# Bill9125/T2MS

Hardware: AMD Instinct MI355X
Metric: generated series/sec (B=256, L=96, 1000-step DDPM) (higher is better)
Workload: dtype f32; 1 GPU; configs[1]: DiT denoiser, 1000-step ddpm with CFG (2 forwards/step), B=256/GPU, L=96, cfg_scale=9.0, LA-VAE decode; Philox noise on device; hipGraph=on; sampler lanes=2 (part-batch chains on own streams, include/t2s.h t2s_sampler_set_lanes); global_batch=256, diffusion_steps=1000, parallelism=batch-shard x1, sampler_lanes=2

## Files before the change

t2ms_amd/csrc/t2s_attn.hip:

```cpp
#include <stdlib.h>

#include "t2s_dit_internal.h"

namespace t2s {

struct SoftmaxState {
    float m_run;
    float l_lane;
};

__device__ __forceinline__ float pair_max(float v) {
    const auto r = __builtin_amdgcn_permlane32_swap(__float_as_uint(v), __float_as_uint(v), false, false);
    return fmaxf(__uint_as_float(r[0]), __uint_as_float(r[1]));
}
__device__ __forceinline__ float pair_sum(float v) {
    const auto r = __builtin_amdgcn_permlane32_swap(__float_as_uint(v), __float_as_uint(v), false, false);
    return __uint_as_float(r[0]) + __uint_as_float(r[1]);
}

__device__ __forceinline__ void softmax_block(f32x16& st, f32x16& ot, SoftmaxState& s) {
    float mloc = st[0];
#pragma unroll
    for (int r = 1; r < 16; ++r) mloc = fmaxf(mloc, st[r]);
    mloc = pair_max(mloc);
    const float m_new = fmaxf(s.m_run, mloc);
    const float alpha = __builtin_amdgcn_exp2f(s.m_run - m_new);
    s.m_run = m_new;
    float psum = 0.f;
#pragma unroll
    for (int r = 0; r < 16; ++r) {
        st[r] = __builtin_amdgcn_exp2f(st[r] - m_new);
        psum += st[r];
    }
    s.l_lane = s.l_lane * alpha + psum;
#pragma unroll
    for (int r = 0; r < 16; ++r) ot[r] *= alpha;
}

constexpr float QSCALE = 0.17677669529663687f * 1.4426950408889634f;

constexpr int ATT_SLOTS = 4;
constexpr int ATT_SLOT_F4 = 512;
constexpr int ATT_LDS_BYTES = ATT_SLOTS * ATT_SLOT_F4 * 16;
constexpr int NKB = NTOK / 32;

constexpr float SM_BIG = 1.152921504606847e18f;


struct TileState {
    f32x16 negm;
    float m_ref;
    float l_lane;
};

__device__ __forceinline__ float exp_sum(f32x16& st) {
#pragma unroll
    for (int r = 0; r < 16; ++r) st[r] = __builtin_amdgcn_exp2f(st[r]);
    return ((st[0] + st[1]) + (st[2] + st[3])) + ((st[4] + st[5]) + (st[6] + st[7])) +
           (((st[8] + st[9]) + (st[10] + st[11])) + ((st[12] + st[13]) + (st[14] + st[15])));
}

__device__ __forceinline__ float rereference(const f32x4 (&kf)[4], const f32x4 (&q)[4], f32x16& st,
                                             f32x16& ot, TileState& t) {
#pragma unroll
    for (int r = 0; r < 16; ++r) st[r] = 0.f;
#pragma unroll
    for (int g = 0; g < 4; ++g)
#pragma unroll
        for (int e = 0; e < 4; ++e) st = mfma32(kf[g][e], q[g][e], st);
    float mloc = st[0];
#pragma unroll
    for (int r = 1; r < 16; ++r) mloc = fmaxf(mloc, st[r]);
    mloc = pair_max(mloc);
    const float m_new = fmaxf(t.m_ref, mloc);
    const float alpha = __builtin_amdgcn_exp2f(t.m_ref - m_new);
    t.m_ref = m_new;
    t.l_lane *= alpha;
#pragma unroll
    for (int r = 0; r < 16; ++r) {
        ot[r] *= alpha;
        t.negm[r] = -m_new;
        st[r] -= m_new;
    }
    return exp_sum(st);
}

template <int NT, int NKBT>
__device__ __forceinline__ void attn_packed_body(f32x4* ring, const f32x4* qg, const f32x4* kg,
                                                 const f32x4* vg, f32x4* og, int bh, int t0, int lane,
                                                 int wave) {
    f32x4 qa[4], qb[4];
#pragma unroll
    for (int g = 0; g < 4; ++g) {
        qa[g] = qg[(t0 * 4 + g) * 64 + lane] * QSCALE;
        if (NT == 2) qb[g] = qg[((t0 + 1) * 4 + g) * 64 + lane] * QSCALE;
    }
    f32x16 oa, ob;
    TileState ta, tb;
#pragma unroll
    for (int r = 0; r < 16; ++r) {
        oa[r] = ob[r] = 0.f;
        ta.negm[r] = tb.negm[r] = INFINITY;
    }
    ta.m_ref = tb.m_ref = -INFINITY;
    ta.l_lane = tb.l_lane = 0.f;

    auto issue_clamped = [&](int jb) {
        const int src = jb < NKBT ? jb : NKBT - 1;
        f32x4* slot = ring + (jb & (ATT_SLOTS - 1)) * ATT_SLOT_F4;
        glds16_asm(kg + (src * 4 + wave) * 64 + lane, slot + wave * 64);
        glds16_asm(vg + (src * 4 + wave) * 64 + lane, slot + 256 + wave * 64);
    };
    asm volatile("s_waitcnt vmcnt(4)" ::: "memory");
    __builtin_amdgcn_s_barrier();
    issue_clamped(3);
    f32x4 kf[4];
#pragma unroll
    for (int g = 0; g < 4; ++g) kf[g] = ring[g * 64 + lane];

#pragma unroll 1
    for (int jb = 0; jb < NKBT; ++jb) {
        const f32x4* slot = ring + (jb & (ATT_SLOTS - 1)) * ATT_SLOT_F4 + lane;
        f32x4 vf[4];
#pragma unroll
        for (int g = 0; g < 4; ++g) vf[g] = slot[256 + g * 64];

        f32x16 sta = ta.negm, stb = tb.negm;
        float psa = 0.f, psb = 0.f;
        bool redo = jb == 0;
        if (!redo) {
            sta = mfma32_from(kf[0][0], qa[0][0], ta.negm);
            if (NT == 2) stb = mfma32_from(kf[0][0], qb[0][0], tb.negm);
#pragma unroll
            for (int g = 0; g < 4; ++g)
#pragma unroll
                for (int e = (g == 0 ? 1 : 0); e < 4; ++e) {
                    sta = mfma32(kf[g][e], qa[g][e], sta);
                    if (NT == 2) stb = mfma32(kf[g][e], qb[g][e], stb);
                }
            psa = exp_sum(sta);
            if (NT == 2) psb = exp_sum(stb);
            const bool stale = !(psa < SM_BIG) || !(psb < SM_BIG);
            redo = __builtin_amdgcn_ballot_w64(stale) != 0;
        }
        if (redo) {
            psa = rereference(kf, qa, sta, oa, ta);
            if (NT == 2) psb = rereference(kf, qb, stb, ob, tb);
        }
        ta.l_lane += psa;
        tb.l_lane += psb;
#pragma unroll
        for (int g = 0; g < 4; ++g)
#pragma unroll
            for (int e = 0; e < 4; ++e) oa = mfma32(vf[g][e], sta[4 * g + e], oa);
        asm volatile("s_waitcnt vmcnt(4)" ::: "memory");
        __builtin_amdgcn_s_barrier();
        issue_clamped(jb + 4);
        {
            const f32x4* nslot = ring + ((jb + 1) & (ATT_SLOTS - 1)) * ATT_SLOT_F4 + lane;
#pragma unroll
            for (int g = 0; g < 4; ++g) kf[g] = nslot[g * 64];
        }
        if (NT == 2) {
#pragma unroll
            for (int g = 0; g < 4; ++g)
#pragma unroll
                for (int e = 0; e < 4; ++e) ob = mfma32(vf[g][e], stb[4 * g + e], ob);
        }
    }
    asm volatile("s_waitcnt vmcnt(0)" ::: "memory");

    const int seq = bh / NH, head = bh % NH;
    {
        const float inv = 1.0f / pair_sum(ta.l_lane);
#pragma unroll
        for (int g = 0; g < 4; ++g) {
            const f32x4 w = {oa[4 * g] * inv, oa[4 * g + 1] * inv, oa[4 * g + 2] * inv, oa[4 * g + 3] * inv};
            og[(((size_t)seq * NKBT + t0) * 16 + head * 4 + g) * 64 + lane] = w;
        }
    }
    if (NT == 2) {
        const float inv = 1.0f / pair_sum(tb.l_lane);
#pragma unroll
        for (int g = 0; g < 4; ++g) {
            const f32x4 w = {ob[4 * g] * inv, ob[4 * g + 1] * inv, ob[4 * g + 2] * inv, ob[4 * g + 3] * inv};
            og[(((size_t)seq * NKBT + t0 + 1) * 16 + head * 4 + g) * 64 + lane] = w;
        }
    }
}

template <int PARTS, int TPW, int NKBT>
__device__ __forceinline__ void attn_packed_head(const float* __restrict__ q, const float* __restrict__ k,
                                                 const float* __restrict__ vT, float* __restrict__ o, int BH) {
    extern __shared__ __attribute__((aligned(16))) f32x4 ring[];
    const int grp = blockIdx.x / (8 * PARTS), rr = blockIdx.x % (8 * PARTS);
    const int bh = grp * 8 + (rr & 7);
    const int part = rr >> 3;
    if (bh >= BH) return;
    const int lane = threadIdx.x & 63;
    const int wave = __builtin_amdgcn_readfirstlane(threadIdx.x >> 6);
    const f32x4* qg = reinterpret_cast<const f32x4*>(q) + (size_t)bh * NKBT * 256;
    const f32x4* kg = reinterpret_cast<const f32x4*>(k) + (size_t)bh * NKBT * 256;
    const f32x4* vg = reinterpret_cast<const f32x4*>(vT) + (size_t)bh * NKBT * 256;
    f32x4* og = reinterpret_cast<f32x4*>(o);

    {
        f32x4* slot0 = ring;
        f32x4* slot1 = ring + ATT_SLOT_F4;
        glds16_asm(kg + (0 * 4 + wave) * 64 + lane, slot0 + wave * 64);
        glds16_asm(vg + (0 * 4 + wave) * 64 + lane, slot0 + 256 + wave * 64);
        glds16_asm(kg + (1 * 4 + wave) * 64 + lane, slot1 + wave * 64);
        glds16_asm(vg + (1 * 4 + wave) * 64 + lane, slot1 + 256 + wave * 64);
        f32x4* slot2 = ring + 2 * ATT_SLOT_F4;
        glds16_asm(kg + (2 * 4 + wave) * 64 + lane, slot2 + wave * 64);
        glds16_asm(vg + (2 * 4 + wave) * 64 + lane, slot2 + 256 + wave * 64);
    }
    if constexpr (TPW == 2) {
        const int t0 = part * 8 + wave * 2;
        if (t0 + 1 < NKBT) {
            attn_packed_body<2, NKBT>(ring, qg, kg, vg, og, bh, t0, lane, wave);
        } else if constexpr (PARTS * 8 > NKBT + 1) {
            attn_packed_body<1, NKBT>(ring, qg, kg, vg, og, bh, t0 < NKBT ? t0 : NKBT - 1, lane, wave);
        } else {
            attn_packed_body<1, NKBT>(ring, qg, kg, vg, og, bh, t0, lane, wave);
        }
    } else {
        const int t = part * 4 + wave;
        attn_packed_body<1, NKBT>(ring, qg, kg, vg, og, bh, t < NKBT ? t : NKBT - 1, lane, wave);
    }
}

template <int PARTS>
__global__ __launch_bounds__(256, 2) void attn_fwd_packed_kernel(const float* __restrict__ q,
                                                                 const float* __restrict__ k,
                                                                 const float* __restrict__ vT,
                                                                 float* __restrict__ o, int BH) {
    attn_packed_head<PARTS, PARTS == 2 ? 2 : 1, NKB>(q, k, vT, o, BH);
}

template <int NKBT>
__global__ __launch_bounds__(256, 2) void attn_fwd_packed_wide_kernel(const float* __restrict__ q,
                                                                      const float* __restrict__ k,
                                                                      const float* __restrict__ vT,
                                                                      float* __restrict__ o, int BH) {
    static_assert(NKBT > 24 && NKBT <= 32, "four workgroups of 8 tile slots");
    attn_packed_head<4, 2, NKBT>(q, k, vT, o, BH);
}

constexpr int PERSIST_THREADS = 512;

template <int NT>
__device__ __forceinline__ void attn_persistent_body(f32x4* ring, const f32x4* qall, const f32x4* kall,
                                                     const f32x4* vall, f32x4* og, int BH, int lane, int wave) {
    const int stride = gridDim.x;
    const int t0 = wave * 2;
    auto issue_block = [&](int bh, int jb, int gslot) {
        if constexpr (NT == 1) {
            if (jb >= NKB) { jb -= NKB; bh += stride; }
            if (bh >= BH) { bh -= stride; jb = NKB - 1; }
            const size_t off = (size_t)bh * NKB * 256 + jb * 4 * 64 + lane;
            f32x4* dst = ring + (gslot & (ATT_SLOTS - 1)) * ATT_SLOT_F4;
#pragma unroll
            for (int f = 0; f < 4; ++f) {
                glds16_asm(kall + off + f * 64, dst + f * 64);
                glds16_asm(vall + off + f * 64, dst + 256 + f * 64);
            }
        }
    };
#define ATT_PERSIST_WAIT() if constexpr (NT == 1) asm volatile("s_waitcnt vmcnt(16)" ::: "memory")
    int bh = blockIdx.x;
    int gb = 0;
    issue_block(bh, 0, 0);
    issue_block(bh, 1, 1);
    issue_block(bh, 2, 2);

    f32x4 qa[4], qb[4], qna[4], qnb[4];
    {
        const f32x4* qg = qall + (size_t)bh * NKB * 256;
#pragma unroll
        for (int g = 0; g < 4; ++g) {
            qa[g] = qg[(t0 * 4 + g) * 64 + lane] * QSCALE;
            if (NT == 2) qb[g] = qg[((t0 + 1) * 4 + g) * 64 + lane] * QSCALE;
            qna[g] = qa[g];
            qnb[g] = qb[g];
        }
    }
    ATT_PERSIST_WAIT();
    __builtin_amdgcn_s_barrier();
    issue_block(bh, 3, 3);
    f32x4 kf[4];
#pragma unroll
    for (int g = 0; g < 4; ++g) kf[g] = ring[g * 64 + lane];

#pragma unroll 1
    for (; bh < BH; bh += stride) {
        f32x16 oa, ob;
        TileState ta, tb;
#pragma unroll
        for (int r = 0; r < 16; ++r) {
            oa[r] = ob[r] = 0.f;
            ta.negm[r] = tb.negm[r] = INFINITY;
        }
        ta.m_ref = tb.m_ref = -INFINITY;
        ta.l_lane = tb.l_lane = 0.f;

#pragma unroll 1
        for (int jb = 0; jb < NKB; ++jb, ++gb) {
            const f32x4* slot = ring + (gb & (ATT_SLOTS - 1)) * ATT_SLOT_F4 + lane;
            f32x4 vf[4];
#pragma unroll
            for (int g = 0; g < 4; ++g) vf[g] = slot[256 + g * 64];
            f32x16 sta = ta.negm, stb = tb.negm;
            float psa = 0.f, psb = 0.f;
            bool redo = jb == 0;
            if (!redo) {
                sta = mfma32_from(kf[0][0], qa[0][0], ta.negm);
                if (NT == 2) stb = mfma32_from(kf[0][0], qb[0][0], tb.negm);
#pragma unroll
                for (int g = 0; g < 4; ++g)
#pragma unroll
                    for (int e = (g == 0 ? 1 : 0); e < 4; ++e) {
                        sta = mfma32(kf[g][e], qa[g][e], sta);
                        if (NT == 2) stb = mfma32(kf[g][e], qb[g][e], stb);
                    }
                psa = exp_sum(sta);
                if (NT == 2) psb = exp_sum(stb);
                const bool stale = !(psa < SM_BIG) || !(psb < SM_BIG);
                redo = __builtin_amdgcn_ballot_w64(stale) != 0;
            }
            if (redo) {
                psa = rereference(kf, qa, sta, oa, ta);
                if (NT == 2) psb = rereference(kf, qb, stb, ob, tb);
            }
            ta.l_lane += psa;
            tb.l_lane += psb;
#pragma unroll
            for (int g = 0; g < 4; ++g)
#pragma unroll
                for (int e = 0; e < 4; ++e) oa = mfma32(vf[g][e], sta[4 * g + e], oa);
            if (jb == NKB - 4 && bh + stride < BH) {
                const f32x4* qg = qall + (size_t)(bh + stride) * NKB * 256;
#pragma unroll
                for (int g = 0; g < 4; ++g) {
                    qna[g] = qg[(t0 * 4 + g) * 64 + lane];
                    if (NT == 2) qnb[g] = qg[((t0 + 1) * 4 + g) * 64 + lane];
                }
            }
            ATT_PERSIST_WAIT();
            __builtin_amdgcn_s_barrier();
            issue_block(bh, jb + 4, gb + 4);
            {
                const f32x4* nslot = ring + ((gb + 1) & (ATT_SLOTS - 1)) * ATT_SLOT_F4 + lane;
#pragma unroll
                for (int g = 0; g < 4; ++g) kf[g] = nslot[g * 64];
            }
            if (NT == 2) {
#pragma unroll
                for (int g = 0; g < 4; ++g)
#pragma unroll
                    for (int e = 0; e < 4; ++e) ob = mfma32(vf[g][e], stb[4 * g + e], ob);
            }
        }
        const int seq = bh / NH, head = bh % NH;
        {
            const float inv = 1.0f / pair_sum(ta.l_lane);
#pragma unroll
            for (int g = 0; g < 4; ++g) {
                const f32x4 w = {oa[4 * g] * inv, oa[4 * g + 1] * inv, oa[4 * g + 2] * inv, oa[4 * g + 3] * inv};
                og[(((size_t)seq * NKB + t0) * 16 + head * 4 + g) * 64 + lane] = w;
            }
        }
        if (NT == 2) {
            const float inv = 1.0f / pair_sum(tb.l_lane);
#pragma unroll
            for (int g = 0; g < 4; ++g) {
                const f32x4 w = {ob[4 * g] * inv, ob[4 * g + 1] * inv, ob[4 * g + 2] * inv, ob[4 * g + 3] * inv};
                og[(((size_t)seq * NKB + t0 + 1) * 16 + head * 4 + g) * 64 + lane] = w;
            }
        }
#pragma unroll
        for (int g = 0; g < 4; ++g) {
            qa[g] = qna[g] * QSCALE;
            if (NT == 2) qb[g] = qnb[g] * QSCALE;
        }
    }
    asm volatile("s_waitcnt vmcnt(0)" ::: "memory");
}

__global__ __launch_bounds__(PERSIST_THREADS, 2) void attn_fwd_persistent_kernel(
    const float* __restrict__ q, const float* __restrict__ k, const float* __restrict__ vT,
    float* __restrict__ o, int BH) {
    extern __shared__ __attribute__((aligned(16))) f32x4 ring[];
    const int lane = threadIdx.x & 63;
    const int wave = __builtin_amdgcn_readfirstlane(threadIdx.x >> 6);
    const f32x4* qg = reinterpret_cast<const f32x4*>(q);
    const f32x4* kg = reinterpret_cast<const f32x4*>(k);
    const f32x4* vg = reinterpret_cast<const f32x4*>(vT);
    f32x4* og = reinterpret_cast<f32x4*>(o);
    if (wave < 7)
        attn_persistent_body<2>(ring, qg, kg, vg, og, BH, lane, wave);
    else
        attn_persistent_body<1>(ring, qg, kg, vg, og, BH, lane, wave);
}

int launch_attn_packed(const float* q, const float* k, const float* vT, float* o, int BH, hipStream_t st) {
    static int n_cu = 0;
    if (n_cu == 0) {
        int dev = 0;
        hipDeviceProp_t prop;
        if (hipGetDevice(&dev) == hipSuccess && hipGetDeviceProperties(&prop, dev) == hipSuccess)
            n_cu = prop.multiProcessorCount;
        else
            n_cu = 256;
    }
    static const int persist_min = getenv("T2S_ATTN_PERSIST_MIN") ? atoi(getenv("T2S_ATTN_PERSIST_MIN")) : 0;
    if (BH >= (persist_min > 0 ? persist_min : 3 * n_cu)) {
        attn_fwd_persistent_kernel<<<BH < n_cu ? BH : n_cu, PERSIST_THREADS, ATT_LDS_BYTES, st>>>(q, k, vT, o, BH);
    } else {
        static const int parts_env = getenv("T2S_ATTN_PARTS") ? atoi(getenv("T2S_ATTN_PARTS")) : 0;
        const int parts = parts_env == 2 || parts_env == 4 ? parts_env : (((BH + 7) / 8) * 16 < n_cu ? 4 : 2);
        if (parts == 4)
            attn_fwd_packed_kernel<4><<<((BH + 7) / 8) * 32, 256, ATT_LDS_BYTES, st>>>(q, k, vT, o, BH);
        else
            attn_fwd_packed_kernel<2><<<((BH + 7) / 8) * 16, 256, ATT_LDS_BYTES, st>>>(q, k, vT, o, BH);
    }
    T2S_LAUNCH_CHECK();
    return T2S_OK;
}

constexpr int KSTR = 36;
constexpr int PLAIN_LDS_BYTES = (NTOK * KSTR + NTOK * DH) * 4;

__global__ __launch_bounds__(512) void attn_fwd_plain_kernel(const float* __restrict__ q,
                                                             const float* __restrict__ k,
                                                             const float* __restrict__ v,
                                                             float* __restrict__ o) {
    extern __shared__ __attribute__((aligned(16))) float smem[];
    float* Ks = smem;
    float* Vs = smem + NTOK * KSTR;
    const int bh = blockIdx.x;
    const int tid = threadIdx.x;
    const int lane = tid & 63, wave = tid >> 6, half = lane >> 5, i = lane & 31;
    const float* kg = k + (size_t)bh * NTOK * DH;
    const float* vg = v + (size_t)bh * NTOK * DH;
    const float* qg = q + (size_t)bh * NTOK * DH;
    for (int idx = tid; idx < NTOK * DH / 4; idx += 512) {
        const f32x4 kv = reinterpret_cast<const f32x4*>(kg)[idx];
        const f32x4 vv = reinterpret_cast<const f32x4*>(vg)[idx];
        const int row = idx >> 3, col = (idx & 7) * 4;
        *reinterpret_cast<f32x4*>(Ks + row * KSTR + col) = kv;
        *reinterpret_cast<f32x4*>(Vs + row * DH + col) = vv;
    }
    __syncthreads();
    for (int qt = wave; qt < NKB; qt += 8) {
        f32x4 qf[4];
#pragma unroll
        for (int g = 0; g < 4; ++g)
            qf[g] = *reinterpret_cast<const f32x4*>(qg + (size_t)(qt * 32 + i) * DH + 8 * g + 4 * half) * QSCALE;
        f32x16 ot;
#pragma unroll
        for (int r = 0; r < 16; ++r) ot[r] = 0.f;
        SoftmaxState s{-INFINITY, 0.f};
        for (int jb = 0; jb < NKB; ++jb) {
            f32x16 st;
#pragma unroll
            for (int r = 0; r < 16; ++r) st[r] = 0.f;
            const float* krow = Ks + (jb * 32 + i) * KSTR + 4 * half;
#pragma unroll
            for (int g = 0; g < 4; ++g) {
                const f32x4 kf = *reinterpret_cast<const f32x4*>(krow + 8 * g);
#pragma unroll
                for (int e = 0; e < 4; ++e) st = mfma32(kf[e], qf[g][e], st);
            }
            softmax_block(st, ot, s);
            const float* vrow = Vs + (jb * 32 + 4 * half) * DH + i;
#pragma unroll
            for (int r = 0; r < 16; ++r) {
                const int klo = (r & 3) + 8 * (r >> 2);
                ot = mfma32(vrow[klo * DH], st[r], ot);
            }
        }
        const float inv = 1.0f / pair_sum(s.l_lane);
#pragma unroll
        for (int g = 0; g < 4; ++g) {
            const f32x4 w = {ot[4 * g] * inv, ot[4 * g + 1] * inv, ot[4 * g + 2] * inv, ot[4 * g + 3] * inv};
            *reinterpret_cast<f32x4*>(o + ((size_t)bh * NTOK + qt * 32 + i) * DH + 8 * g + 4 * half) = w;
        }
    }
}

int launch_attn_packed_n(const float* q, const float* k, const float* vT, float* o, int BH, int n_tok, hipStream_t st) {
    if (n_tok == NTOK) return launch_attn_packed(q, k, vT, o, BH, st);
    const int grid = ((BH + 7) / 8) * 32;
    if (n_tok == 800) {
        attn_fwd_packed_wide_kernel<25><<<grid, 256, ATT_LDS_BYTES, st>>>(q, k, vT, o, BH);
    } else if (n_tok == 1024) {
        attn_fwd_packed_wide_kernel<32><<<grid, 256, ATT_LDS_BYTES, st>>>(q, k, vT, o, BH);
    } else {
        set_error("attention: n_tok=%d (480, 800 or 1024)", n_tok);
        return T2S_E_INVALID;
    }
    T2S_LAUNCH_CHECK();
    return T2S_OK;
}

int attn_init() {
    static bool attr_set = false;
    if (!attr_set) {
        T2S_HIP_CHECK(hipFuncSetAttribute(reinterpret_cast<const void*>(attn_fwd_plain_kernel),
                                          hipFuncAttributeMaxDynamicSharedMemorySize, PLAIN_LDS_BYTES));
        attr_set = true;
    }
    return T2S_OK;
}

}

extern "C" int t2s_attn_fwd(const float* q, const float* k, const float* v, float* o, int BH,
                            void* stream) {
    T2S_REQUIRE(q && k && v && o, "t2s_attn_fwd: NULL pointer");
    T2S_REQUIRE(BH > 0, "t2s_attn_fwd: BH=%d must be > 0", BH);
    if (int rc = t2s::attn_init()) return rc;
    t2s::attn_fwd_plain_kernel<<<BH, 512, t2s::PLAIN_LDS_BYTES, (hipStream_t)stream>>>(q, k, v, o);
    T2S_LAUNCH_CHECK();
    return T2S_OK;
}


extern "C" int t2s_attn_fwd_packed(const float* q, const float* k, const float* vT, float* o, int n_seq,
                                   void* stream) {
    T2S_REQUIRE(q && k && vT && o, "t2s_attn_fwd_packed: NULL pointer");
    T2S_REQUIRE(n_seq > 0, "t2s_attn_fwd_packed: n_seq=%d must be > 0", n_seq);
    return t2s::launch_attn_packed(q, k, vT, o, n_seq * t2s::NH, (hipStream_t)stream);
}

extern "C" int t2s_attn_fwd_packed_n(const float* q, const float* k, const float* vT, float* o, int n_seq, int n_tok,
                                     void* stream) {
    T2S_REQUIRE(q && k && vT && o, "t2s_attn_fwd_packed_n: NULL pointer");
    T2S_REQUIRE(n_seq > 0 && n_seq <= (1 << 20), "t2s_attn_fwd_packed_n: n_seq=%d out of range", n_seq);
    T2S_REQUIRE(n_tok == 480 || n_tok == 800 || n_tok == 1024, "t2s_attn_fwd_packed_n: n_tok=%d must be 480, 800 or 1024", n_tok);
    return t2s::launch_attn_packed_n(q, k, vT, o, n_seq * t2s::NH, n_tok, (hipStream_t)stream);
}
```

Measured before the change: 64.58 series/s.

## Add quad-head persistent attention kernel balancing tiles across waves

Adds a persistent attention kernel that walks heads in groups of four. It reassigns query tiles across the eight waves so the last wave, which previously handled a single tile per head, shares work drawn from neighbouring heads. Each wave's K/V ring is doubled in LDS and gets a second staging region, and an LDS flag exchange coordinates rescaling for the split-tile form. The kernel is used when each block gets at least four heads, and can be turned off with an environment variable. The trade-off is double the LDS footprint and more complex control flow and synchronisation per key block, in exchange for removing wave idle time.

```diff
diff --git a/t2ms_amd/csrc/t2s_attn.hip b/t2ms_amd/csrc/t2s_attn.hip
--- a/t2ms_amd/csrc/t2s_attn.hip
+++ b/t2ms_amd/csrc/t2s_attn.hip
@@ -403,6 +403,294 @@
         attn_persistent_body<1>(ring, qg, kg, vg, og, BH, lane, wave);
 }
 
+constexpr int QUAD_RING_F4 = ATT_SLOTS * ATT_SLOT_F4;
+constexpr int QUAD_LDS_BYTES = 2 * ATT_LDS_BYTES + 2 * 8 * 4;
+enum { QV_PAIR, QV_ONE, QV_ONEX, QV_TWO };
+enum { QP_PLAIN = 4 };
+
+struct QuadSlots {
+    int ha, ta, ra;
+    int hb, tb, rb;
+};
+
+template <int N>
+struct QuadForm {
+    static constexpr int value = N;
+};
+
+template <int ROLE>
+__device__ __forceinline__ void attn_quad_walk(f32x4* lds, const f32x4* qall, const f32x4* kall, const f32x4* vall,
+                                               f32x4* og, int BH, int lane, int wave) {
+    const int stride = gridDim.x, first = blockIdx.x;
+    const int n = (BH - first + stride - 1) / stride;
+    const int nq4 = n & ~3;
+    const unsigned flag_base = (unsigned)(size_t)((__attribute__((address_space(3))) char*)(lds + 2 * QUAD_RING_F4));
+    auto ptype = [&](int p) { return p < nq4 ? (p & 3) : (int)QP_PLAIN; };
+    auto slots = [&](int p) {
+        const int t = ptype(p), hm = first + p * stride;
+        QuadSlots s;
+        s.ha = s.hb = hm;
+        s.ta = 2 * wave;
+        s.tb = 2 * wave + 1;
+        s.ra = s.rb = 0;
+        if (ROLE == 1 && t == 3) s.ta = s.tb = wave + 4;
+        if (ROLE == 2) {
+            s.ta = s.tb = NKB - 1;
+            if (t == 0) { s.hb = hm + 3 * stride; s.rb = QUAD_RING_F4; }
+            if (t == 1) { s.ha = s.hb = hm + 2 * stride; s.ta = 12; s.tb = 13; s.ra = s.rb = QUAD_RING_F4; }
+            if (t == 2) { s.hb = hm - stride; s.rb = QUAD_RING_F4; }
+            if (t == 3) s.ta = s.tb = 11;
+        }
+        return s;
+    };
+
+    const f32x4* const piece_src = (wave < 4 ? kall : vall) + (wave & 3) * 64 + lane;
+    int ip = 0, ij = 0, islot = 0;
+    auto issue_next = [&]() {
+        const int ph = ip < n ? ip : n - 1, pj = ip < n ? ij : NKB - 1;
+        f32x4* dst = lds + islot * ATT_SLOT_F4 + wave * 64;
+        glds16_asm(piece_src + ((size_t)(first + ph * stride) * NKB + pj) * 256, dst);
+        const int t = ptype(ip);
+        if (t < 3) {
+            const int hs = first + (ip + (t == 0 ? 3 : (t == 1 ? 2 : -1))) * stride;
+            glds16_asm(piece_src + ((size_t)hs * NKB + ij) * 256, dst + QUAD_RING_F4);
+        }
+        islot = (islot + 1) & (ATT_SLOTS - 1);
+        if (++ij == NKB) { ij = 0; ++ip; }
+    };
+    auto wait_ring = [&]() { asm volatile("s_waitcnt vmcnt(2) lgkmcnt(0)" ::: "memory"); };
+    issue_next();
+    issue_next();
+    issue_next();
+
+    QuadSlots cur = slots(0);
+    f32x4 qa[4], qb[4], qna[4], qnb[4];
+#pragma unroll
+    for (int g = 0; g < 4; ++g) {
+        qa[g] = qall[((size_t)cur.ha * NKB + cur.ta) * 256 + g * 64 + lane] * QSCALE;
+        qb[g] = qall[((size_t)cur.hb * NKB + cur.tb) * 256 + g * 64 + lane] * QSCALE;
+        qna[g] = qa[g];
+        qnb[g] = qb[g];
+    }
+    wait_ring();
+    __builtin_amdgcn_s_barrier();
+    f32x4 kf[4];
+#pragma unroll
+    for (int g = 0; g < 4; ++g) kf[g] = lds[cur.ra + g * 64 + lane];
+    int gb = 0;
+
+    auto store_tile = [&](const f32x16& o, const TileState& t, int bh, int tile) {
+        const int seq = bh / NH, head = bh % NH;
+        const float inv = 1.0f / pair_sum(t.l_lane);
+#pragma unroll
+        for (int g = 0; g < 4; ++g) {
+            const f32x4 w = {o[4 * g] * inv, o[4 * g + 1] * inv, o[4 * g + 2] * inv, o[4 * g + 3] * inv};
+            og[(((size_t)seq * NKB + tile) * 16 + head * 4 + g) * 64 + lane] = w;
+        }
+    };
+
+    auto run_pass = [&](auto form, const QuadSlots nxt, const bool has_next) {
+        constexpr int V = decltype(form)::value;
+        constexpr bool TWO_TILES = V == QV_PAIR || V == QV_TWO;
+        f32x16 oa, ob;
+        TileState ta, tb;
+#pragma unroll
+        for (int r = 0; r < 16; ++r) {
+            oa[r] = ob[r] = 0.f;
+            ta.negm[r] = tb.negm[r] = INFINITY;
+        }
+        ta.m_ref = tb.m_ref = -INFINITY;
+        ta.l_lane = tb.l_lane = 0.f;
+
+        int jb = 0;
+#pragma unroll 1
+        for (int run = 0; run < 2; ++run) {
+        const int jend = run == 0 ? NKB - 4 : NKB;
+#pragma unroll 1
+        for (; jb < jend; ++jb, ++gb) {
+            const int soff = (gb & (ATT_SLOTS - 1)) * ATT_SLOT_F4 + lane;
+            f32x4 vf[4];
+#pragma unroll
+            for (int g = 0; g < 4; ++g) vf[g] = lds[cur.ra + soff + 256 + g * 64];
+            const bool take_q = jb == NKB - 4 && has_next;
+            auto land_q = [&]() {
+                if (take_q) {
+#pragma unroll
+                    for (int g = 0; g < 4; ++g) {
+                        qna[g] = qna[g] * QSCALE;
+                        qnb[g] = qnb[g] * QSCALE;
+                        asm volatile("" : "+v"(qna[g]), "+v"(qnb[g]));
+                    }
+                }
+            };
+            auto next_k = [&]() {
+                const int noff = ((gb + 1) & (ATT_SLOTS - 1)) * ATT_SLOT_F4 + lane;
+                const int kra = jb < NKB - 1 ? cur.ra : nxt.ra;
+#pragma unroll
+                for (int g = 0; g < 4; ++g) kf[g] = lds[kra + noff + g * 64];
+            };
+            f32x16 sta = ta.negm, stb = tb.negm;
+            float psa = 0.f, psb = 0.f;
+
+            if constexpr (V == QV_ONEX) {
+                unsigned mine = 1;
+                if (jb != 0) {
+                    sta = mfma32_from(kf[0][0], qa[0][0], ta.negm);
+#pragma unroll
+                    for (int g = 0; g < 4; ++g)
+#pragma unroll
+                        for (int e = (g == 0 ? 1 : 0); e < 4; ++e) sta = mfma32(kf[g][e], qa[g][e], sta);
+                    psa = exp_sum(sta);
+                    mine = __builtin_amdgcn_ballot_w64(!(psa < SM_BIG)) != 0;
+                }
+                issue_next();
+                const unsigned fset = flag_base + (jb & 1) * 32;
+                asm volatile("ds_write_b32 %0, %1\n\ts_waitcnt lgkmcnt(0)" ::"v"(fset + wave * 4), "v"(mine) : "memory");
+                land_q();
+                wait_ring();
+                __builtin_amdgcn_s_barrier();
+                unsigned theirs;
+                asm volatile("ds_read_b32 %0, %1\n\ts_waitcnt lgkmcnt(0)" : "=&v"(theirs) : "v"(fset + (wave ^ 1) * 4) : "memory");
+                if (mine | __builtin_amdgcn_readfirstlane(theirs)) psa = rereference(kf, qa, sta, oa, ta);
+                ta.l_lane += psa;
+                next_k();
+#pragma unroll
+                for (int g = 0; g < 4; ++g)
+#pragma unroll
+                    for (int e = 0; e < 4; ++e) oa = mfma32(vf[g][e], sta[4 * g + e], oa);
+            } else if constexpr (V == QV_TWO) {
+                auto scores = [&](const f32x4(&qx)[4], f32x16& st, f32x16& ot, TileState& tx) {
+                    float ps = 0.f;
+                    bool redo = jb == 0;
+                    if (jb != 0) {
+                        st = mfma32_from(kf[0][0], qx[0][0], tx.negm);
+#pragma unroll
+                        for (int g = 0; g < 4; ++g)
+#pragma unroll
+                            for (int e = (g == 0 ? 1 : 0); e < 4; ++e) st = mfma32(kf[g][e], qx[g][e], st);
+                        ps = exp_sum(st);
+                        redo = __builtin_amdgcn_ballot_w64(!(ps < SM_BIG)) != 0;
+                    }
+                    if (redo) ps = rereference(kf, qx, st, ot, tx);
+                    tx.l_lane += ps;
+                };
+                scores(qa, sta, oa, ta);
+                issue_next();
+                asm volatile("" ::: "memory");
+#pragma unroll
+                for (int g = 0; g < 4; ++g) kf[g] = lds[cur.rb + soff + g * 64];
+#pragma unroll
+                for (int g = 0; g < 4; ++g)
+#pragma unroll
+                    for (int e = 0; e < 4; ++e) oa = mfma32(vf[g][e], sta[4 * g + e], oa);
+                asm volatile("" ::: "memory");
+#pragma unroll
+                for (int g = 0; g < 4; ++g) vf[g] = lds[cur.rb + soff + 256 + g * 64];
+                scores(qb, stb, ob, tb);
+                land_q();
+                wait_ring();
+                __builtin_amdgcn_s_barrier();
+                next_k();
+#pragma unroll
+                for (int g = 0; g < 4; ++g)
+#pragma unroll
+                    for (int e = 0; e < 4; ++e) ob = mfma32(vf[g][e], stb[4 * g + e], ob);
+            } else {
+                bool redo = jb == 0;
+                if (!redo) {
+                    sta = mfma32_from(kf[0][0], qa[0][0], ta.negm);
+                    if (TWO_TILES) stb = mfma32_from(kf[0][0], qb[0][0], tb.negm);
+#pragma unroll
+                    for (int g = 0; g < 4; ++g)
+#pragma unroll
+                        for (int e = (g == 0 ? 1 : 0); e < 4; ++e) {
+                            sta = mfma32(kf[g][e], qa[g][e], sta);
+                            if (TWO_TILES) stb = mfma32(kf[g][e], qb[g][e], stb);
+                        }
+                    psa = exp_sum(sta);
+                    if (TWO_TILES) psb = exp_sum(stb);
+                    const bool stale = !(psa < SM_BIG) || !(psb < SM_BIG);
+                    redo = __builtin_amdgcn_ballot_w64(stale) != 0;
+                }
+                issue_next();
+                if (redo) {
+                    psa = rereference(kf, qa, sta, oa, ta);
+                    if (TWO_TILES) psb = rereference(kf, qb, stb, ob, tb);
+                }
+                ta.l_lane += psa;
+                tb.l_lane += psb;
+#pragma unroll
+                for (int g = 0; g < 4; ++g)
+#pragma unroll
+                    for (int e = 0; e < 4; ++e) oa = mfma32(vf[g][e], sta[4 * g + e], oa);
+                land_q();
+                wait_ring();
+                __builtin_amdgcn_s_barrier();
+                next_k();
+                if (TWO_TILES) {
+#pragma unroll
+                    for (int g = 0; g < 4; ++g)
+#pragma unroll
+                        for (int e = 0; e < 4; ++e) ob = mfma32(vf[g][e], stb[4 * g + e], ob);
+                }
+            }
+        }
+        if (run == 0 && has_next) {
+#pragma unroll
+            for (int g = 0; g < 4; ++g) {
+                qna[g] = qall[((size_t)nxt.ha * NKB + nxt.ta) * 256 + g * 64 + lane];
+                qnb[g] = qall[((size_t)nxt.hb * NKB + nxt.tb) * 256 + g * 64 + lane];
+            }
+        }
+        }
+        store_tile(oa, ta, cur.ha, cur.ta);
+        if (TWO_TILES) store_tile(ob, tb, cur.hb, cur.tb);
+#pragma unroll
+        for (int g = 0; g < 4; ++g) {
+            qa[g] = qna[g];
+            qb[g] = qnb[g];
+        }
+    };
+
+#pragma unroll 1
+    for (int p = 0; p < n; ++p) {
+        const bool has_next = p + 1 < n;
+        const QuadSlots nxt = has_next ? slots(p + 1) : cur;
+        const int t = ptype(p);
+        if constexpr (ROLE == 0) {
+            run_pass(QuadForm<QV_PAIR>{}, nxt, has_next);
+        } else if constexpr (ROLE == 1) {
+            if (t == 3) run_pass(QuadForm<QV_ONEX>{}, nxt, has_next);
+            else run_pass(QuadForm<QV_PAIR>{}, nxt, has_next);
+        } else {
+            if (t == QP_PLAIN) run_pass(QuadForm<QV_ONE>{}, nxt, has_next);
+            else if (t == 3) run_pass(QuadForm<QV_ONEX>{}, nxt, has_next);
+            else if (t == 1) run_pass(QuadForm<QV_PAIR>{}, nxt, has_next);
+            else run_pass(QuadForm<QV_TWO>{}, nxt, has_next);
+        }
+        cur = nxt;
+    }
+    asm volatile("s_waitcnt vmcnt(0)" ::: "memory");
+}
+
+__global__ __launch_bounds__(PERSIST_THREADS, 2) void attn_fwd_persistent_quad_kernel(
+    const float* __restrict__ q, const float* __restrict__ k, const float* __restrict__ vT,
+    float* __restrict__ o, int BH) {
+    extern __shared__ __attribute__((aligned(16))) f32x4 ring[];
+    const int lane = threadIdx.x & 63;
+    const int wave = __builtin_amdgcn_readfirstlane(threadIdx.x >> 6);
+    const f32x4* qg = reinterpret_cast<const f32x4*>(q);
+    const f32x4* kg = reinterpret_cast<const f32x4*>(k);
+    const f32x4* vg = reinterpret_cast<const f32x4*>(vT);
+    f32x4* og = reinterpret_cast<f32x4*>(o);
+    if (wave < 4)
+        attn_quad_walk<0>(ring, qg, kg, vg, og, BH, lane, wave);
+    else if (wave < 7)
+        attn_quad_walk<1>(ring, qg, kg, vg, og, BH, lane, wave);
+    else
+        attn_quad_walk<2>(ring, qg, kg, vg, og, BH, lane, wave);
+}
+
 int launch_attn_packed(const float* q, const float* k, const float* vT, float* o, int BH, hipStream_t st) {
     static int n_cu = 0;
     if (n_cu == 0) {
@@ -414,8 +702,17 @@
             n_cu = 256;
     }
     static const int persist_min = getenv("T2S_ATTN_PERSIST_MIN") ? atoi(getenv("T2S_ATTN_PERSIST_MIN")) : 0;
+    static const int grid_cap = getenv("T2S_ATTN_GRID") ? atoi(getenv("T2S_ATTN_GRID")) : 0;
+    static const bool quad_on = !(getenv("T2S_ATTN_QUAD") && atoi(getenv("T2S_ATTN_QUAD")) == 0);
     if (BH >= (persist_min > 0 ? persist_min : 3 * n_cu)) {
-        attn_fwd_persistent_kernel<<<BH < n_cu ? BH : n_cu, PERSIST_THREADS, ATT_LDS_BYTES, st>>>(q, k, vT, o, BH);
+        int grid = BH < n_cu ? BH : n_cu;
+        if (grid_cap > 0 && grid_cap < grid) grid = grid_cap;
+        if (quad_on && BH / grid >= 4) {
+            if (int rc = attn_init()) return rc;
+            attn_fwd_persistent_quad_kernel<<<grid, PERSIST_THREADS, QUAD_LDS_BYTES, st>>>(q, k, vT, o, BH);
+        } else {
+            attn_fwd_persistent_kernel<<<grid, PERSIST_THREADS, ATT_LDS_BYTES, st>>>(q, k, vT, o, BH);
+        }
     } else {
         static const int parts_env = getenv("T2S_ATTN_PARTS") ? atoi(getenv("T2S_ATTN_PARTS")) : 0;
         const int parts = parts_env == 2 || parts_env == 4 ? parts_env : (((BH + 7) / 8) * 16 < n_cu ? 4 : 2);
@@ -509,6 +806,8 @@
     if (!attr_set) {
         T2S_HIP_CHECK(hipFuncSetAttribute(reinterpret_cast<const void*>(attn_fwd_plain_kernel),
                                           hipFuncAttributeMaxDynamicSharedMemorySize, PLAIN_LDS_BYTES));
+        T2S_HIP_CHECK(hipFuncSetAttribute(reinterpret_cast<const void*>(attn_fwd_persistent_quad_kernel),
+                                          hipFuncAttributeMaxDynamicSharedMemorySize, QUAD_LDS_BYTES));
         attr_set = true;
     }
     return T2S_OK;
```

Result: faster. 65.23 series/s, median of 6 (+1.0%).
